# ziqin-h/GIVEPose

Hardware: AMD Instinct MI355X
Metric: images/sec PoseNet fwd, bs=64 256x256 fp16, 1/2/4/8 MI355X; % MFMA roofline (higher is better)
Workload: dtype f16

## Files before the change

### givepose_amd/csrc/gemm.hip

```cpp
#include "common.hpp"

namespace {

struct GemmKP {
    const void* X;
    const void* W;
    const float* bias;
    const float* gamma;
    const void* res;
    void* C;
    float* ws;
    int M, N, K, ldx, ldc, ldres, epi, out_f32;
    int conv, H, Win, Cin, KW, stride, pad, Ho, Wo;
    int tiles_m, tiles_n, nkt, kt_per_split, splitk;
    float* gn_partial;
    int gn_cpg, gn_hw;
    int early;
    const float* ln_stats;
    const float* ln_s;
    int ln_nsl;
    float ln_eps;
    int dbg;
    const char* pf;
    long pf_bytes;
// ... 326 lines not shown
            if (!PRE) {
#pragma unroll
                for (int i = i0; i < i0 + 4; ++i) {
                    const int m = mb + j * 32 + i * 4 + er;
                    for (int e = 0; e < 4; ++e) r4[0][i][e] = 0;
                    if (sres && nok && m < p.M) r4[0][i] = load_res4<RT>(p, m, en);
                }
            }
#pragma unroll
            for (int i = i0; i < i0 + 4; ++i) {
                const int row = i * 4 + er, chunk = lane & 15;
                const f32x4 v = *reinterpret_cast<const f32x4*>(slab + row * 256 + ((chunk ^ (row & 7)) << 4));
                const int m = mb + j * 32 + row;
                if (m < p.M && nok) {
                    const f32x4 o = epi_apply<RT>(epi_code, v, b4, g4, r4[PRE ? j : 0][i]);
                    if (SPL && p.out_planes) {
                        half4 hv, lv;
#pragma unroll
                        for (int e = 0; e < 4; ++e) {
                            hv[e] = (half_t)o[e];
                            lv[e] = (half_t)((o[e] - (float)hv[e]) * p.split_up);
                        }
                        half_t* ch = reinterpret_cast<half_t*>(p.C) + (long)m * p.ldc + en;
                        *reinterpret_cast<half4*>(ch) = hv;
                        *reinterpret_cast<half4*>(ch + p.cplane) = lv;
                    } else
                    if (p.dbg != 4 || o[0] == 12345.678f) store4<RT>(p, m, en, o);
                    if (p.c16) {
                        half4 hv;
#pragma unroll
                        for (int e = 0; e < 4; ++e) hv[e] = (half_t)o[e];
                        *reinterpret_cast<half4*>(reinterpret_cast<half_t*>(p.c16) + (long)m * p.ldc16 + en) = hv;
                    }
                    gsum += (o[0] + o[1]) + (o[2] + o[3]);
                    gsq += (o[0] * o[0] + o[1] * o[1]) + (o[2] * o[2] + o[3] * o[3]);
                }
            }
        }
        if (p.gn_partial && (j & 1)) {
            float a = gsum, q = gsq;
            a += __shfl_xor(a, 16, 64); q += __shfl_xor(q, 16, 64);
            a += __shfl_xor(a, 32, 64); q += __shfl_xor(q, 32, 64);
            if (p.gn_cpg == 8) { a += __shfl_xor(a, 1, 64); q += __shfl_xor(q, 1, 64); }
            const int mrow = mb + (j - 1) * 32;
            if (er == 0 && nok && mrow < p.M && (p.gn_cpg == 4 || (lane & 1) == 0)) {
                const int G = p.N / p.gn_cpg, cpi = p.gn_hw >> 6;
                const int b = mrow / p.gn_hw, ch = (mrow - b * p.gn_hw) >> 6;
                float* o = p.gn_partial + (((long)b * cpi + ch) * G + en / p.gn_cpg) * 2;
                o[0] = a;
                o[1] = q;
            }
            gsum = gsq = 0.f;
        }
    }
}

template <int MT, int NT>
__device__ __forceinline__ void epilogue_split(const GemmKP& p, f32x4 (&acc)[NT][MT], char* slab, int mb, int nb, int lane) {
    switch (p.epi) {
        case GP_EPI_GELU: epilogue_generic<float, MT, NT, true, GP_EPI_GELU>(p, acc, slab, mb, nb, lane); break;
        case GP_EPI_RELU: epilogue_generic<float, MT, NT, true, GP_EPI_RELU>(p, acc, slab, mb, nb, lane); break;
        case GP_EPI_LRELU: epilogue_generic<float, MT, NT, true, GP_EPI_LRELU>(p, acc, slab, mb, nb, lane); break;
        case GP_EPI_SCALE_RES: epilogue_generic<float, MT, NT, true, GP_EPI_SCALE_RES>(p, acc, slab, mb, nb, lane); break;
        case GP_EPI_RES_RELU: epilogue_generic<float, MT, NT, true, GP_EPI_RES_RELU>(p, acc, slab, mb, nb, lane); break;
        default: epilogue_generic<float, MT, NT, true, GP_EPI_NONE>(p, acc, slab, mb, nb, lane); break;
    }
}

template <typename T, int WM, int WN, int MT, int NT, int NS, bool DB = false, int RB = 128, bool PP = false, bool SPL = false, bool R32 = false>
__global__ __launch_bounds__(WM * WN * 64, WM * WN == 4 ? 2 : 1) void gemm_big_kernel(const GemmKP pin) {
    static_assert(NT == 4, "epilogue slab assumes a 64-wide wave tile");
    static_assert(!SPL || sizeof(T) == 2, "split-operand mode: fp16 planes");
    static_assert(!R32 || (sizeof(T) == 2 && !SPL), "R32: fp16 operands with an fp32 residual / output");
    typedef typename std::conditional<SPL || R32, float, T>::type RT;
    GemmKP p = pin;
    int kt0 = 0;
    if constexpr (!PP && !(DB && NS == 2)) {
        if (pin.splitk > 1) {
            kt0 = blockIdx.y * pin.kt_per_split;
            p.nkt = min(pin.nkt - kt0, pin.kt_per_split);
            p.C = reinterpret_cast<float*>(pin.C) + (long)blockIdx.y * pin.M * pin.N;
        }
    }
    static_assert(!PP || (WM * WN == 8 && (NS == 4 || NS == 5) && RB == 64 && !DB), "ping-pong schedule: 8 waves, 4/5-stage ring of 64-byte K steps");
    constexpr int NW = WM * WN;
    constexpr int BM = WM * MT * 16, BN = WN * NT * 16;
    static_assert(RB == 128 || (RB == 64 && !DB), "RB");
    constexpr int EPT = 16 / sizeof(T), KPT = RB / sizeof(T), CPR = RB / 16, RPI = 1024 / RB;
    constexpr int XI = BM / RPI / NW, WI = BN / RPI / NW;
    constexpr int STAGE = (BM + BN) * RB;
    static_assert(NS * STAGE >= NW * 8192, "epilogue slabs must fit");
    __shared__ __attribute__((aligned(1024))) char smem[NS * STAGE];

    const int tid = threadIdx.x, lane = tid & 63;
    const int wave = __builtin_amdgcn_readfirstlane(tid >> 6);
    const int wm = wave % WM, wn = wave / WM;

    const int nblk = p.tiles_m * p.tiles_n;
    const int bid = blockIdx.x;
    const int q = nblk >> 3, r8 = nblk & 7, xcd = bid & 7, idx = bid >> 3;
    const int tile = (xcd < r8 ? xcd * (q + 1) : r8 * (q + 1) + (xcd - r8) * q) + idx;
    const int tm = tile / p.tiles_n, tn = tile - tm * p.tiles_n;
    const int m0 = tm * BM, n0 = tn * BN;
    const PfSink pfs = prefetch_issue(p, bid + blockIdx.y * gridDim.x, gridDim.x * gridDim.y, wave, WM * WN, lane);

    const T* __restrict__ X = reinterpret_cast<const T*>(p.X);
    const T* __restrict__ W = reinterpret_cast<const T*>(p.W);
    const T* zero = reinterpret_cast<const T*>(gp_zero_page_tu);

    const int lrow = lane / CPR;
    const int lchunk = RB == 128 ? ((lane & 7) ^ (lrow & 7)) : ((lane & 3) ^ ((-(lrow >> 2)) & 3));
    const char* xptr[XI];
    unsigned xmask[XI];
    const char* wptr[WI];
#pragma unroll
    for (int i = 0; i < XI; ++i) {
        const int m = m0 + (i * NW + wave) * RPI + lrow;
        const bool ok = m < p.M;
        if (p.conv) {
            const int hw = p.Ho * p.Wo;
            const int b = m / hw, r = m - b * hw;
            const int ho = r / p.Wo, wo = r - ho * p.Wo;
            const int hi0 = ho * p.stride - p.pad, wi0 = wo * p.stride - p.pad;
            xptr[i] = reinterpret_cast<const char*>(X + (((long)b * p.H + hi0) * p.Win + wi0) * p.Cin + lchunk * EPT);
            unsigned mk = 0;
            const int KH = p.K / (p.KW * p.Cin);
            for (int kh = 0; kh < KH; ++kh)
                for (int kw = 0; kw < p.KW; ++kw)
                    if (ok && (unsigned)(hi0 + kh) < (unsigned)p.H && (unsigned)(wi0 + kw) < (unsigned)p.Win)
                        mk |= 1u << (kh * p.KW + kw);
            xmask[i] = mk;
        } else {
            xptr[i] = reinterpret_cast<const char*>(X + (long)m * p.ldx + lchunk * EPT);
            xmask[i] = ok ? 1u : 0u;
        }
    }
#pragma unroll
    for (int i = 0; i < WI; ++i) {
        const int n = n0 + (i * NW + wave) * RPI + lrow;
        wptr[i] = n < p.N ? reinterpret_cast<const char*>(W + (long)n * p.K + lchunk * EPT) : nullptr;
    }
    const int cpt = p.conv ? p.Cin / KPT : 1;

    const unsigned lds0 = (unsigned)(size_t)(lds_char_t*)smem;
    auto stage = [&](int buf, int kt) {
        const unsigned xs = lds0 + buf * STAGE + wave * 1024;
        const unsigned ws = xs + BM * RB;
        long xoff;
        unsigned bit = 1u;
        kt += kt0;
        long xadd = 0, wadd = 0;
        if constexpr (SPL) {
            const int seg = (kt >= p.split_n1 ? 1 : 0) + (kt >= 2 * p.split_n1 ? 1 : 0);
            kt -= seg * p.split_n1;
            xadd = seg == 1 ? p.xplane_b : 0;
            wadd = seg == 0 ? p.wplane_b : 0;
        }
        if (p.conv) {
            const int tap = kt / cpt;
            const int kh = tap / p.KW, kw = tap - kh * p.KW;
            xoff = (((long)kh * p.Win + kw) * p.Cin + (kt - tap * cpt) * KPT) * (long)sizeof(T);
            bit = 1u << tap;
        } else {
            xoff = (long)kt * RB;
        }
        const char* zp = reinterpret_cast<const char*>(zero);
#pragma unroll
// ... 2 lines not shown
        for (int i = 0; i < WI; ++i) glds16(wptr[i] ? wptr[i] + (long)kt * RB + wadd : zp, ws + i * NW * 1024);
    };

    bool lean = false;
    if constexpr (sizeof(T) == 2 && !SPL) {
        const bool res_epi = p.epi == GP_EPI_SCALE_RES || p.epi == GP_EPI_RES_RELU;
        lean = !p.out_f32 && p.dbg != 5 && m0 + BM <= p.M && n0 + BN <= p.N && p.ldc % 8 == 0 &&
               ((size_t)p.C & 15) == 0 && !(res_epi && (p.gn_partial || p.ldres % 8 || ((size_t)p.res & 15)));
    }
    f32x4 acc[NT][MT];
#pragma unroll
    for (int a = 0; a < NT; ++a) {
        f32x4 init = f32x4{0.f, 0.f, 0.f, 0.f};
        if (lean && p.bias && p.epi != GP_EPI_LNFOLD_GELU) init = *reinterpret_cast<const f32x4*>(p.bias + n0 + wn * NT * 16 + a * 16 + (lane >> 4) * 4);
#pragma unroll
        for (int b = 0; b < MT; ++b) acc[a][b] = init;
    }
    auto split_rescale = [&](int kt) {
        if constexpr (SPL) {
            if (kt + kt0 == 2 * p.split_n1) {
#pragma unroll
                for (int a = 0; a < NT; ++a)
#pragma unroll
                    for (int b = 0; b < MT; ++b) acc[a][b] *= p.split_scale;
            }
        }
    };

    const int fr = lane & 15, fq = lane >> 4, sw = fr & 7;
    const int xfo = (wm * MT * 16 + fr) * RB, wfo = (wn * NT * 16 + fr) * RB;
    auto compute = [&](int buf) {
        const char* xs = smem + buf * STAGE + xfo;
        const char* ws = smem + buf * STAGE + BM * RB + wfo;
        if constexpr (RB == 64) {
            const int co = (fq ^ ((-(fr >> 2)) & 3)) << 4;
            uint4 xf[MT], wf[NT];
#pragma unroll
            for (int t = 0; t < NT; ++t) wf[t] = *reinterpret_cast<const uint4*>(ws + t * 1024 + co);
#pragma unroll
            for (int t = 0; t < MT; ++t) xf[t] = *reinterpret_cast<const uint4*>(xs + t * 1024 + co);
#pragma unroll
            for (int mt = 0; mt < MT; ++mt)
#pragma unroll
                for (int nt = 0; nt < NT; ++nt) mma<T>(acc[nt][mt], wf[nt], xf[mt]);
        } else if constexpr (DB) {
            const int co0 = ((0 * 4 + fq) ^ sw) << 4, co1 = ((1 * 4 + fq) ^ sw) << 4;
            uint4 xf0[MT], wf0[NT], xf1[MT], wf1[NT];
#pragma unroll
            for (int t = 0; t < NT; ++t) wf0[t] = *reinterpret_cast<const uint4*>(ws + t * 2048 + co0);
#pragma unroll
            for (int t = 0; t < MT; ++t) xf0[t] = *reinterpret_cast<const uint4*>(xs + t * 2048 + co0);
#pragma unroll
            for (int t = 0; t < NT; ++t) wf1[t] = *reinterpret_cast<const uint4*>(ws + t * 2048 + co1);
#pragma unroll
            for (int t = 0; t < MT; ++t) xf1[t] = *reinterpret_cast<const uint4*>(xs + t * 2048 + co1);
            __builtin_amdgcn_s_setprio(1);
#pragma unroll
            for (int mt = 0; mt < MT; ++mt)
#pragma unroll
                for (int nt = 0; nt < NT; ++nt) mma<T>(acc[nt][mt], wf0[nt], xf0[mt]);
#pragma unroll
            for (int mt = 0; mt < MT; ++mt)
#pragma unroll
                for (int nt = 0; nt < NT; ++nt) mma<T>(acc[nt][mt], wf1[nt], xf1[mt]);
            __builtin_amdgcn_s_setprio(0);
        } else {
#pragma unroll
            for (int ks = 0; ks < 2; ++ks) {
                const int co = ((ks * 4 + fq) ^ sw) << 4;
                uint4 xf[MT], wf[NT];
#pragma unroll
                for (int t = 0; t < NT; ++t) wf[t] = *reinterpret_cast<const uint4*>(ws + t * 2048 + co);
#pragma unroll
                for (int t = 0; t < MT; ++t) xf[t] = *reinterpret_cast<const uint4*>(xs + t * 2048 + co);
#pragma unroll
                for (int mt = 0; mt < MT; ++mt)
#pragma unroll
                    for (int nt = 0; nt < NT; ++nt) mma<T>(acc[nt][mt], wf[nt], xf[mt]);
            }
        }
    };

    constexpr int G = XI + WI;
    if constexpr (PP) {
        constexpr int LEAD = NS - 2;
        const int grp = wave >> 2;
        const int co = (fq ^ ((-(fr >> 2)) & 3)) << 4;
        uint4 xf[MT], wf[NT];
        const bool sdma = !p.conv && (long)BM * p.ldx * sizeof(T) < (1l << 31) && (long)BN * p.K * sizeof(T) < (1l << 31);
        unsigned xo[XI], wo[WI];
#pragma unroll
        for (int i = 0; i < XI; ++i) {
            const int r = min((i * NW + wave) * RPI + lrow, p.M - 1 - m0);
            xo[i] = (unsigned)(((long)r * p.ldx + lchunk * EPT) * sizeof(T));
        }
#pragma unroll
        for (int i = 0; i < WI; ++i) {
            const int r = min((i * NW + wave) * RPI + lrow, p.N - 1 - n0);
            wo[i] = (unsigned)(((long)r * p.K + lchunk * EPT) * sizeof(T));
        }
        const char* xtile = reinterpret_cast<const char*>(X + (long)m0 * p.ldx);
        const char* wtile = reinterpret_cast<const char*>(W + (long)n0 * p.K);
        auto stage_s = [&](int buf, int kt) {
            const unsigned xs = lds0 + buf * STAGE + wave * 1024;
            const unsigned ws = xs + BM * RB;
            long xadd = 0, wadd = 0;
            if constexpr (SPL) {
                const int seg = (kt >= p.split_n1 ? 1 : 0) + (kt >= 2 * p.split_n1 ? 1 : 0);
                kt -= seg * p.split_n1;
                xadd = seg == 1 ? p.xplane_b : 0;
                wadd = seg == 0 ? p.wplane_b : 0;
            }
            const char* bx = xtile + (long)kt * RB + xadd;
            const char* bw = wtile + (long)kt * RB + wadd;
#pragma unroll
            for (int i = 0; i < XI; ++i) glds16_s(bx, xo[i], xs + i * NW * 1024);
#pragma unroll
            for (int i = 0; i < WI; ++i) glds16_s(bw, wo[i], ws + i * NW * 1024);
        };
#pragma unroll
        for (int i = 0; i < LEAD; ++i)
            if (i < p.nkt) { if (sdma) stage_s(i, i); else stage(i, i); }
        if constexpr (LEAD == 3) {
            if (p.nkt >= 3) asm volatile("s_waitcnt vmcnt(%0)" ::"n"(2 * G) : "memory");
            else if (p.nkt == 2) asm volatile("s_waitcnt vmcnt(%0)" ::"n"(G) : "memory");
            else asm volatile("s_waitcnt vmcnt(0)" ::: "memory");
        } else {
            if (p.nkt >= 2) asm volatile("s_waitcnt vmcnt(%0)" ::"n"(G) : "memory");
            else asm volatile("s_waitcnt vmcnt(0)" ::: "memory");
        }
        prefetch_retire(pfs);
        __builtin_amdgcn_s_barrier();
        if (grp) __builtin_amdgcn_s_barrier();
        int buf = 0, nbuf = LEAD;
        clk_stamp(p, 0);
#ifdef GP_PP_STAMPS
#define GP_PPS(k)                                                                                                              \
        do {                                                                                                                     \
            if (p.ws && p.splitk <= 1 && blockIdx.x == 0 && (wave & 3) == 0 && lane == 0 && kt >= 8 && kt < 24) {                  \
                __builtin_amdgcn_sched_barrier(0);                                                                               \
                unsigned long long t_;                                                                                           \
                asm volatile("s_memtime %0\n\ts_waitcnt lgkmcnt(0)" : "=s"(t_) :: "memory");                                    \
                reinterpret_cast<unsigned long long*>(p.ws)[4096 + ((wave >> 2) * 16 + (kt - 8)) * 8 + (k)] = t_;                 \
                __builtin_amdgcn_sched_barrier(0);                                                                               \
            }                                                                                                                    \
        } while (0)
#else
#define GP_PPS(k) do {} while (0)
#endif
        for (int kt = 0; kt < p.nkt; ++kt) {
            GP_PPS(0);
            if (p.dbg != 2) {
                const char* xs = smem + buf * STAGE + xfo;
                const char* ws = smem + buf * STAGE + BM * RB + wfo;
#pragma unroll
                for (int t = 0; t < NT; ++t) wf[t] = *reinterpret_cast<const uint4*>(ws + t * 1024 + co);
#pragma unroll
                for (int t = 0; t < MT; ++t) xf[t] = *reinterpret_cast<const uint4*>(xs + t * 1024 + co);
            }
            __builtin_amdgcn_sched_barrier(0);
            GP_PPS(1);
            if (kt + LEAD < p.nkt && (p.dbg != 1 || kt + LEAD < NS)) { if (sdma) stage_s(nbuf, kt + LEAD); else stage(nbuf, kt + LEAD); }
            GP_PPS(2);
            if (LEAD == 3 && kt + 3 < p.nkt) asm volatile("s_waitcnt vmcnt(%0)" ::"n"(2 * G) : "memory");
            else if (kt + 2 < p.nkt) asm volatile("s_waitcnt vmcnt(%0)" ::"n"(G) : "memory");
            else asm volatile("s_waitcnt vmcnt(0)" ::: "memory");
// ... 1098 lines not shown
    }
    GP_SM(KMAX);
#undef GP_SM
}


template <int MR>
__global__ __launch_bounds__(256) void gemv_kernel(const GemmKP p) {
    constexpr int KC = 4096, NCH = KC / 512;
    __shared__ __attribute__((aligned(16))) half_t xs[MR][KC];
    const int tid = threadIdx.x, lane = tid & 63, wave = tid >> 6;
    const int n0 = blockIdx.x * 8 + wave * 2;
    const half_t* X = reinterpret_cast<const half_t*>(p.X);
    const half_t* W0 = reinterpret_cast<const half_t*>(p.W) + (long)n0 * p.K + lane * 8;
    float acc[MR][2];
#pragma unroll
    for (int m = 0; m < MR; ++m) acc[m][0] = acc[m][1] = 0.f;
    for (int k0 = 0; k0 < p.K; k0 += KC) {
        const int kc = min(KC, p.K - k0), nch = kc >> 9;
        uint4 w[2][NCH];
#pragma unroll
        for (int j = 0; j < NCH; ++j)
            if (j < nch) {
                w[0][j] = *reinterpret_cast<const uint4*>(W0 + k0 + j * 512);
                w[1][j] = *reinterpret_cast<const uint4*>(W0 + p.K + k0 + j * 512);
            }
        if (k0) __syncthreads();
        for (int i = tid; i < MR * (kc >> 3); i += 256) {
            const int m = i / (kc >> 3), c = i - m * (kc >> 3);
            uint4 v = uint4{0u, 0u, 0u, 0u};
            if (m < p.M) v = *reinterpret_cast<const uint4*>(X + (long)m * p.ldx + k0 + c * 8);
            *reinterpret_cast<uint4*>(&xs[m][c * 8]) = v;
        }
        __syncthreads();
#pragma unroll
        for (int j = 0; j < NCH; ++j)
            if (j < nch) {
#pragma unroll
                for (int m = 0; m < MR; ++m) {
                    const uint4 xv = *reinterpret_cast<const uint4*>(&xs[m][j * 512 + lane * 8]);
                    const unsigned xw[4] = {xv.x, xv.y, xv.z, xv.w};
#pragma unroll
                    for (int c = 0; c < 2; ++c) {
                        const unsigned ww[4] = {w[c][j].x, w[c][j].y, w[c][j].z, w[c][j].w};
#pragma unroll
                        for (int e = 0; e < 4; ++e)
                            acc[m][c] = __builtin_amdgcn_fdot2(__builtin_bit_cast(half2v, xw[e]), __builtin_bit_cast(half2v, ww[e]), acc[m][c], false);
                    }
                }
            }
    }
#pragma unroll
    for (int m = 0; m < MR; ++m)
#pragma unroll
        for (int c = 0; c < 2; ++c)
#pragma unroll
            for (int o = 32; o >= 1; o >>= 1) acc[m][c] += __shfl_xor(acc[m][c], o, 64);
    if (lane == 0) {
        const f32x4 z = f32x4{0.f, 0.f, 0.f, 0.f};
#pragma unroll
        for (int m = 0; m < MR; ++m)
            if (m < p.M) {
                const f32x4 b = p.bias ? f32x4{p.bias[n0], p.bias[n0 + 1], 0.f, 0.f} : z;
                const f32x4 v = epi_apply<half_t>(p.epi, f32x4{acc[m][0], acc[m][1], 0.f, 0.f}, b, z, half4{0, 0, 0, 0});
                if (p.out_f32) {
                    float* o = reinterpret_cast<float*>(p.C) + (long)m * p.ldc + n0;
                    o[0] = v[0];
                    o[1] = v[1];
                } else {
                    half_t* o = reinterpret_cast<half_t*>(p.C) + (long)m * p.ldc + n0;
                    o[0] = (half_t)v[0];
                    o[1] = (half_t)v[1];
                }
            }
    }
}

}

static bool pp_enabled() {
    static const bool on = [] { const char* e = getenv("GP_GEMM_PP"); return !(e && e[0] == '0'); }();
    return on;
}

static bool conv_wide_enabled() {
    static const bool on = [] { const char* e = getenv("GP_CONV_WIDE"); return !(e && e[0] == '0'); }();
    return on;
}

static bool conv_window_enabled() {
    static const bool on = [] { const char* e = getenv("GP_CONV_WINDOW"); return !(e && e[0] == '0'); }();
    return on;
}

static long pp_min_k() {
    static const long k = [] { const char* e = getenv("GP_PP_MIN_K"); return e ? atol(e) : 512l; }();
    return k;
}

static int gp_num_cus() {
    static const int n = [] {
        int dev = 0, cu = 0;
        if (hipGetDevice(&dev) != hipSuccess || hipDeviceGetAttribute(&cu, hipDeviceAttributeMultiprocessorCount, dev) != hipSuccess || cu <= 0) cu = 256;
        return cu;
    }();
    return n;
}

static bool prefetch_enabled() {
    static const bool on = [] { const char* e = getenv("GP_GEMM_PREFETCH"); return !(e && e[0] == '0'); }();
    return on;
}

static bool wreg_enabled() {
    static const bool on = [] { const char* e = getenv("GP_GEMM_WREG"); return !(e && e[0] == '0'); }();
    return on;
}
static bool wreg_early() {
    static const bool on = [] { const char* e = getenv("GP_GEMM_WREG_EARLY"); return !(e && e[0] == '0'); }();
    return on;
}
static long wreg_min_rows() {
    static const long k = [] { const char* e = getenv("GP_GEMM_WREG_MIN_ROWS"); return e ? atol(e) : 6144l; }();
    return k;
}

static int wreg_variant() {
    static const int v = [] { const char* e = getenv("GP_GEMM_WREG_VARIANT"); const int x = e ? atoi(e) : (gp_gelu16_enabled() ? 21 : 22); return (x >= 19 && x <= 22) ? x : 17; }();
    return v;
}

static long co_min_tiles() {
    static const long k = [] { const char* e = getenv("GP_GEMM_CO_MIN_TILES"); return e ? atol(e) : 32l; }();
    return k;
}

static double smallm_tile_bias() {
    static const double b = [] { const char* e = getenv("GP_GEMM_SMALLM_BIAS"); return e ? atof(e) : 0.0; }();
    return b;
}
static double smallm_estimate(int M, int N, int K, int mt) {
    const double wgs = (double)(M / (16 * mt)) * (N / 32), kb_per_wg = (16.0 * mt + 32.0) * K * 2.0 / 1024.0;
    const double one = 1.0 + kb_per_wg / 60.0, many = wgs / 256.0 * kb_per_wg / 45.0;
    return 2.6 + (one > many ? one : many) + (mt == 4 ? 1.5 : 0.0);
}

static bool gemv_enabled() {
    static const bool on = [] { const char* e = getenv("GP_GEMM_GEMV"); return !(e && e[0] == '0'); }();
    return on;
}

static int smallm_max_rows() {
    static const int n = [] { const char* e = getenv("GP_GEMM_SMALLM_MAXROWS"); return e && atoi(e) > 0 ? atoi(e) : 16384; }();
    return n;
}

static bool smallm_enabled() {
    static const bool on = [] { const char* e = getenv("GP_GEMM_SMALLM"); return !(e && e[0] == '0'); }();
    return on;
}

static long pp_min_tiles() {
    const char* e = getenv("GP_GEMM_PP_MIN_TILES");
    return e ? atol(e) : 192;
}

// ... 188 lines not shown
        switch (d->epilogue) {
            case GP_EPI_GELU:
#ifdef GP_WREG_STAMPS
                if (p.dbg == 16 && p.ws) { hipLaunchKernelGGL((gemm_wreg_kernel<GP_EPI_GELU, 16>), dim3(grid), dim3(512), 0, s, p); break; }
                if (p.dbg == 1) { hipLaunchKernelGGL((gemm_wreg_kernel<GP_EPI_GELU, 1>), dim3(grid), dim3(512), 0, s, p); break; }
                if (p.dbg == 2) { hipLaunchKernelGGL((gemm_wreg_kernel<GP_EPI_GELU, 2>), dim3(grid), dim3(512), 0, s, p); break; }
                if (p.dbg == 4) { hipLaunchKernelGGL((gemm_wreg_kernel<GP_EPI_GELU, 4>), dim3(grid), dim3(512), 0, s, p); break; }
                if (p.dbg == 8) { hipLaunchKernelGGL((gemm_wreg_kernel<GP_EPI_NONE, 8>), dim3(grid), dim3(512), 0, s, p); break; }
                if (p.dbg == 10) { hipLaunchKernelGGL((gemm_wreg_kernel<GP_EPI_NONE, 10>), dim3(grid), dim3(512), 0, s, p); break; }
                if (p.dbg == 14) { hipLaunchKernelGGL((gemm_wreg_kernel<GP_EPI_NONE, 14>), dim3(grid), dim3(512), 0, s, p); break; }
#endif
                hipLaunchKernelGGL(gemm_wreg_kernel<GP_EPI_GELU>, dim3(grid), dim3(512), 0, s, p);
                break;
            case GP_EPI_RELU: hipLaunchKernelGGL(gemm_wreg_kernel<GP_EPI_RELU>, dim3(grid), dim3(512), 0, s, p); break;
            case GP_EPI_LRELU: hipLaunchKernelGGL(gemm_wreg_kernel<GP_EPI_LRELU>, dim3(grid), dim3(512), 0, s, p); break;
            default: hipLaunchKernelGGL(gemm_wreg_kernel<GP_EPI_NONE>, dim3(grid), dim3(512), 0, s, p); break;
        }
        GP_LAUNCH_CHECK("gp_gemm");
    }
    if (variant == 17) {
        GP_REQUIRE(wreg_ok && d->ldc % 8 == 0 && ((size_t)d->C & 15) == 0, "gp_gemm: variant 17 needs a plain fp16 GEMM with K = 512, N %% 256 == 0, M %% 32 == 0, ldc %% 8 == 0, "
                   "16-byte aligned C, epilogue none/gelu/relu/lrelu");
        const int nsl = d->N / 256, tiles = d->M / 32;
        const int want = gp_num_cus() / nsl > 0 ? gp_num_cus() / nsl : 1;
        p.tiles_m = cdiv(tiles, want);
        const int groups = cdiv(tiles, p.tiles_m);
        const int grid = cdiv(groups * nsl, 8) * 8;
        switch (d->epilogue) {
            case GP_EPI_GELU: hipLaunchKernelGGL(gemm_wreg2_kernel<GP_EPI_GELU>, dim3(grid), dim3(512), 0, s, p); break;
            case GP_EPI_RELU: hipLaunchKernelGGL(gemm_wreg2_kernel<GP_EPI_RELU>, dim3(grid), dim3(512), 0, s, p); break;
            case GP_EPI_LRELU: hipLaunchKernelGGL(gemm_wreg2_kernel<GP_EPI_LRELU>, dim3(grid), dim3(512), 0, s, p); break;
            default: hipLaunchKernelGGL(gemm_wreg2_kernel<GP_EPI_NONE>, dim3(grid), dim3(512), 0, s, p); break;
        }
        GP_LAUNCH_CHECK("gp_gemm");
    }
    if (variant >= 19 && variant <= 22) {
        GP_REQUIRE(wreg_ok && d->ldc % 8 == 0 && ((size_t)d->C & 15) == 0, "gp_gemm: variant 19-22 needs a plain fp16 GEMM with K = 512, N %% 256 == 0, M %% 32 == 0, ldc %% 8 == 0, "
                   "16-byte aligned C, epilogue none/gelu/relu/lrelu");
        const int nsl = d->N / 256, tiles = d->M / 32;
        const int want = gp_num_cus() / nsl > 0 ? gp_num_cus() / nsl : 1;
        p.tiles_m = cdiv(tiles, want);
        const int groups = cdiv(tiles, p.tiles_m);
        const int grid = cdiv(groups * nsl, 8) * 8;
        const bool s32 = variant <= 20, g16 = variant == 20 || variant == 21;
#define GP_W3(E, S, G) hipLaunchKernelGGL((gemm_wreg3_kernel<E, S, G>), dim3(grid), dim3(512), 0, s, p)
        switch (d->epilogue) {
            case GP_EPI_GELU:
                if (s32) { if (g16) GP_W3(GP_EPI_GELU, 1, 1); else GP_W3(GP_EPI_GELU, 1, 0); }
                else { if (g16) GP_W3(GP_EPI_GELU, 0, 1); else GP_W3(GP_EPI_GELU, 0, 0); }
                break;
            case GP_EPI_RELU: if (s32) GP_W3(GP_EPI_RELU, 1, 0); else GP_W3(GP_EPI_RELU, 0, 0); break;
            case GP_EPI_LRELU: if (s32) GP_W3(GP_EPI_LRELU, 1, 0); else GP_W3(GP_EPI_LRELU, 0, 0); break;
            default: if (s32) GP_W3(GP_EPI_NONE, 1, 0); else GP_W3(GP_EPI_NONE, 0, 0); break;
        }
#undef GP_W3
        GP_LAUNCH_CHECK("gp_gemm");
    }
    if (variant == 13) {
        GP_REQUIRE(win_ok, "gp_gemm: variant 13 needs a 3x3 s1 p1 fp16 conv with Cout 256, W in {64, 32, 16}");
        p.tiles_m = d->M / 256;
        p.tiles_n = 1;
        const bool wide = !split && d->Win >= 32 && d->M % 512 == 0 && d->H % (512 / d->Win) == 0 && p.dbg != 9 && (p.dbg == 8 || conv_wide_enabled());
        if (split) {
            if (d->Win == 64) hipLaunchKernelGGL((conv3_pp_kernel<64, 4, true>), dim3(p.tiles_m), dim3(512), 0, s, p);
            else if (d->Win == 32) hipLaunchKernelGGL((conv3_pp_kernel<32, 4, true>), dim3(p.tiles_m), dim3(512), 0, s, p);
            else hipLaunchKernelGGL((conv3_pp_kernel<16, 4, true>), dim3(p.tiles_m), dim3(512), 0, s, p);
        }
#ifdef GP_CONV_GNL
        else if (d->Win == 64 && p.dbg == 7) hipLaunchKernelGGL((conv3_pp_kernel<64, 4, false, true>), dim3(p.tiles_m), dim3(512), 0, s, p);
        else if (d->Win == 32 && p.dbg == 7) hipLaunchKernelGGL((conv3_pp_kernel<32, 4, false, true>), dim3(p.tiles_m), dim3(512), 0, s, p);
#endif
        else if (wide && d->Win == 64) { p.tiles_m = d->M / 512; hipLaunchKernelGGL((conv3_pp_kernel<64, 4, false, false, true>), dim3(p.tiles_m * 2), dim3(512), 0, s, p); }
        else if (wide && d->Win == 32) { p.tiles_m = d->M / 512; hipLaunchKernelGGL((conv3_pp_kernel<32, 4, false, false, true>), dim3(p.tiles_m * 2), dim3(512), 0, s, p); }
        else if (d->Win == 64) hipLaunchKernelGGL((conv3_pp_kernel<64, 4>), dim3(p.tiles_m), dim3(512), 0, s, p);
        else if (d->Win == 32) hipLaunchKernelGGL((conv3_pp_kernel<32, 4>), dim3(p.tiles_m), dim3(512), 0, s, p);
        else hipLaunchKernelGGL((conv3_pp_kernel<16, 4>), dim3(p.tiles_m), dim3(512), 0, s, p);
        GP_LAUNCH_CHECK("gp_gemm");
    }
    if (variant == 12) {
        if (d->dtype == GP_F16) launch_big<half_t, 2, 4, 8, 4, 5, false, 64, true>(p, s); else launch_big<float, 2, 2, 4, 4, 2>(p, s);
        GP_LAUNCH_CHECK("gp_gemm");
    }
    if (variant == 10) {
        if (split) launch_big<half_t, 2, 4, 8, 4, 4, false, 64, true, true>(p, s);
        else if (r32) launch_big<half_t, 2, 4, 8, 4, 4, false, 64, true, false, true>(p, s);
        else if (d->dtype == GP_F16) launch_big<half_t, 2, 4, 8, 4, 4, false, 64, true>(p, s); else launch_big<float, 2, 2, 4, 4, 2>(p, s);
        GP_LAUNCH_CHECK("gp_gemm");
    }
    if (variant == 11) {
        if (d->dtype == GP_F16) launch_big<half_t, 2, 4, 4, 4, 4, false, 64, true>(p, s); else launch_big<float, 2, 2, 4, 4, 2>(p, s);
        GP_LAUNCH_CHECK("gp_gemm");
    }
    if (variant == 8) {
        if (split) launch_big<half_t, 2, 2, 8, 4, 3, false, 64, false, true>(p, s);
        else if (d->dtype == GP_F16) launch_big<half_t, 2, 2, 8, 4, 3, false, 64>(p, s); else launch_big<float, 2, 2, 4, 4, 2>(p, s);
        GP_LAUNCH_CHECK("gp_gemm");
    }
    if (variant == 9) {
        if (d->dtype == GP_F16) launch_big<half_t, 2, 2, 8, 4, 4, false, 64>(p, s); else launch_big<float, 2, 2, 4, 4, 2>(p, s);
        GP_LAUNCH_CHECK("gp_gemm");
    }
    if (variant == 7) {
        if (split) launch_big<half_t, 2, 2, 4, 4, 2, true, 128, false, true>(p, s);
        else if (r32) launch_big<half_t, 2, 2, 4, 4, 2, true, 128, false, false, true>(p, s);
        else if (d->dtype == GP_F16) launch_big<half_t, 2, 2, 4, 4, 2, true>(p, s); else launch_big<float, 2, 2, 4, 4, 2>(p, s);
        GP_LAUNCH_CHECK("gp_gemm");
    }
    if (variant == 5) {
        if (d->dtype == GP_F16) launch_big<half_t, 2, 2, 4, 4, 4>(p, s); else launch_big<float, 2, 2, 4, 4, 4>(p, s);
        GP_LAUNCH_CHECK("gp_gemm");
    }
    if (variant == 4) {
        if (p.splitk > 1) {
            GemmKP q = p;
            q.C = d->workspace; q.out_f32 = 1; q.ldc = d->N; q.epi = GP_EPI_NONE; q.bias = nullptr; q.gamma = nullptr; q.res = nullptr;
            if (split) launch_big<half_t, 2, 2, 4, 4, 2, false, 128, false, true>(q, s);
            else if (d->dtype == GP_F16) launch_big<half_t, 2, 2, 4, 4, 2>(q, s); else launch_big<float, 2, 2, 4, 4, 2>(q, s);
            p.splitk = q.splitk;
            const long work = (long)d->M * (d->N / 4);
            if (d->dtype == GP_F16 && !split) hipLaunchKernelGGL(splitk_reduce_kernel<half_t>, dim3(cdiv(work, 256)), dim3(256), 0, s, p);
            else hipLaunchKernelGGL(splitk_reduce_kernel<float>, dim3(cdiv(work, 256)), dim3(256), 0, s, p);
            GP_LAUNCH_CHECK("gp_gemm");
        }
        if (split) launch_big<half_t, 2, 2, 4, 4, 2, false, 128, false, true>(p, s);
        else if (d->dtype == GP_F16) launch_big<half_t, 2, 2, 4, 4, 2>(p, s); else launch_big<float, 2, 2, 4, 4, 2>(p, s);
        GP_LAUNCH_CHECK("gp_gemm");
    }
    if (variant == 3) {
        if (d->dtype == GP_F16) launch_big<half_t, 2, 4, 8, 4, 2>(p, s); else launch_big<float, 2, 2, 4, 4, 2>(p, s);
        GP_LAUNCH_CHECK("gp_gemm");
    }
    if (variant == 2) {
        if (d->dtype == GP_F16) launch_big<half_t, 4, 2, 4, 4, 3>(p, s); else launch_big<float, 4, 2, 4, 4, 3>(p, s);
        GP_LAUNCH_CHECK("gp_gemm");
    }
    return gp_fail(GP_ERR_INVALID, "gp_gemm: variant %d not handled", variant);
}
```

Measured before the change: 12800.

## Add eight-phase ping-pong GEMM schedule with double-buffered 128-byte K steps

Adds a new ping-pong path to the big fp16 GEMM kernel. It runs on two LDS buffers of 128-byte K steps, split into half-tiles, and works through four compute quadrants per K tile. Fragment reads, global-to-LDS staging and MFMA bursts are interleaved under barriers and priority hints. Plain fp16 GEMMs with K >= 1024 use it by default, with an environment switch and debug overrides. The goal is to hide more load latency and cut barrier overhead per K step, at the cost of more registers, a tighter schedule and more code paths.

```diff
diff --git a/givepose_amd/csrc/gemm.hip b/givepose_amd/csrc/gemm.hip
--- a/givepose_amd/csrc/gemm.hip
+++ b/givepose_amd/csrc/gemm.hip
@@ -432,7 +432,8 @@
             p.C = reinterpret_cast<float*>(pin.C) + (long)blockIdx.y * pin.M * pin.N;
         }
     }
-    static_assert(!PP || (WM * WN == 8 && (NS == 4 || NS == 5) && RB == 64 && !DB), "ping-pong schedule: 8 waves, 4/5-stage ring of 64-byte K steps");
+    static_assert(!PP || (WM * WN == 8 && (NS == 4 || NS == 5) && RB == 64 && !DB) || (WM == 2 && WN == 4 && MT == 8 && NS == 2 && RB == 128 && !DB && !SPL && !R32 && sizeof(T) == 2),
+                  "ping-pong schedule: 8 waves, 4/5-stage ring of 64-byte K steps, or the eight-phase schedule on two buffers of 128-byte K steps");
     constexpr int NW = WM * WN;
     constexpr int BM = WM * MT * 16, BN = WN * NT * 16;
     static_assert(RB == 128 || (RB == 64 && !DB), "RB");
@@ -601,6 +602,110 @@
     };
 
     constexpr int G = XI + WI;
+    if constexpr (PP && RB == 128) {
+        constexpr int HT = 128 * RB;
+        static_assert(STAGE == 4 * HT, "two buffers of four half-tiles");
+        const int grp = wave >> 2;
+        unsigned xo[2][2], wo[2][2];
+#pragma unroll
+        for (int h = 0; h < 2; ++h)
+#pragma unroll
+            for (int j = 0; j < 2; ++j) {
+                const int r = (j * NW + wave) * RPI + lrow;
+                const int xr = min((r >> 6) * 128 + h * 64 + (r & 63), p.M - 1 - m0);
+                const int wr = min((r >> 5) * 64 + h * 32 + (r & 31), p.N - 1 - n0);
+                xo[h][j] = (unsigned)(((long)xr * p.ldx + lchunk * EPT) * sizeof(T));
+                wo[h][j] = (unsigned)(((long)wr * p.K + lchunk * EPT) * sizeof(T));
+            }
+        const char* xtile = reinterpret_cast<const char*>(X + (long)m0 * p.ldx);
+        const char* wtile = reinterpret_cast<const char*>(W + (long)n0 * p.K);
+        auto stage_x = [&](int b, int h, int kt) __attribute__((always_inline)) {
+            const char* bx = xtile + (long)kt * RB;
+            const unsigned ls = lds0 + b * STAGE + h * HT + wave * 1024;
+            glds16_s(bx, xo[h][0], ls);
+            glds16_s(bx, xo[h][1], ls + NW * 1024);
+        };
+        auto stage_w = [&](int b, int h, int kt) __attribute__((always_inline)) {
+            const char* bw = wtile + (long)kt * RB;
+            const unsigned ls = lds0 + b * STAGE + (2 + h) * HT + wave * 1024;
+            glds16_s(bw, wo[h][0], ls);
+            glds16_s(bw, wo[h][1], ls + NW * 1024);
+        };
+        const int co0 = (fq ^ sw) << 4, co1 = ((4 + fq) ^ sw) << 4;
+        const char* xfb = smem + (wm * 64 + fr) * RB;
+        const char* wfb = smem + 2 * HT + (wn * 32 + fr) * RB;
+        uint4 xf[2][4][2], wf[2][2][2];
+        auto read_x = [&](int b, int h) __attribute__((always_inline)) {
+#pragma unroll
+            for (int t = 0; t < 4; ++t) {
+                xf[h][t][0] = *reinterpret_cast<const uint4*>(xfb + b * STAGE + h * HT + t * 16 * RB + co0);
+                xf[h][t][1] = *reinterpret_cast<const uint4*>(xfb + b * STAGE + h * HT + t * 16 * RB + co1);
+            }
+        };
+        auto read_w = [&](int b, int h) __attribute__((always_inline)) {
+#pragma unroll
+            for (int t = 0; t < 2; ++t) {
+                wf[h][t][0] = *reinterpret_cast<const uint4*>(wfb + b * STAGE + h * HT + t * 16 * RB + co0);
+                wf[h][t][1] = *reinterpret_cast<const uint4*>(wfb + b * STAGE + h * HT + t * 16 * RB + co1);
+            }
+        };
+        auto quadrant = [&](int xh, int wh) __attribute__((always_inline)) {
+            __builtin_amdgcn_sched_barrier(0);
+            __builtin_amdgcn_s_barrier();
+            asm volatile("s_waitcnt lgkmcnt(0)" ::: "memory");
+            __builtin_amdgcn_sched_barrier(0);
+            __builtin_amdgcn_s_setprio(1);
+#pragma unroll
+            for (int ks = 0; ks < 2; ++ks)
+#pragma unroll
+                for (int mt = 0; mt < 4; ++mt)
+#pragma unroll
+                    for (int nt = 0; nt < 2; ++nt) mma<T>(acc[wh * 2 + nt][xh * 4 + mt], wf[wh][nt][ks], xf[xh][mt][ks]);
+            __builtin_amdgcn_s_setprio(0);
+            __builtin_amdgcn_sched_barrier(0);
+            __builtin_amdgcn_s_barrier();
+            __builtin_amdgcn_sched_barrier(0);
+        };
+        auto ktile = [&](int b, int kt, bool s1, bool s2) __attribute__((always_inline)) {
+            read_w(b, 0);
+            __builtin_amdgcn_sched_barrier(0);
+            read_x(b, 0);
+            __builtin_amdgcn_sched_barrier(0);
+            if (s1) stage_x(b ^ 1, 1, kt + 1);
+            asm volatile("s_waitcnt lgkmcnt(8)" ::: "memory");
+            quadrant(0, 0);
+            read_w(b, 1);
+            __builtin_amdgcn_sched_barrier(0);
+            if (s2) stage_w(b, 0, kt + 2);
+            quadrant(0, 1);
+            read_x(b, 1);
+            __builtin_amdgcn_sched_barrier(0);
+            if (s2) stage_x(b, 0, kt + 2);
+            quadrant(1, 0);
+            if (s2) {
+                stage_w(b, 1, kt + 2);
+                asm volatile("s_waitcnt vmcnt(6)" ::: "memory");
+            } else {
+                asm volatile("s_waitcnt vmcnt(0)" ::: "memory");
+            }
+            quadrant(1, 1);
+        };
+        stage_x(0, 0, 0); stage_w(0, 0, 0); stage_w(0, 1, 0); stage_x(0, 1, 0);
+        stage_w(1, 0, 1); stage_x(1, 0, 1); stage_w(1, 1, 1);
+        asm volatile("s_waitcnt vmcnt(6)" ::: "memory");
+        prefetch_retire(pfs);
+        __builtin_amdgcn_s_barrier();
+        if (grp) __builtin_amdgcn_s_barrier();
+        clk_stamp(p, 0);
+        for (int kt = 0; kt + 2 < p.nkt; kt += 2) {
+            ktile(0, kt, true, true);
+            ktile(1, kt + 1, true, true);
+        }
+        ktile(0, p.nkt - 2, true, false);
+        ktile(1, p.nkt - 1, false, false);
+        clk_stamp(p, 1);
+        if (!grp) __builtin_amdgcn_s_barrier();
+    } else
     if constexpr (PP) {
         constexpr int LEAD = NS - 2;
         const int grp = wave >> 2;
@@ -1865,6 +1970,13 @@
     static const bool on = [] { const char* e = getenv("GP_GEMM_PP"); return !(e && e[0] == '0'); }();
     return on;
 }
+
+static bool pp128_enabled() {
+    static const bool on = [] { const char* e = getenv("GP_GEMM_PP128"); return !(e && e[0] == '0'); }();
+    return on;
+}
+
+static bool pp128_wins(int K) { return K >= 1024; }
 
 static bool conv_wide_enabled() {
     static const bool on = [] { const char* e = getenv("GP_CONV_WIDE"); return !(e && e[0] == '0'); }();
@@ -2219,6 +2331,21 @@
         GP_LAUNCH_CHECK("gp_gemm");
     }
     if (variant == 10) {
+        const int force = p.dbg == 11 ? 1 : p.dbg == 12 ? -1 : 0;
+        if (force) p.dbg = 0;
+        const bool pp128_ok = d->dtype == GP_F16 && !split && !r32 && d->KH == 0 && d->K % 128 == 0 && d->K >= 256 &&
+                              256l * d->ldx * 2 < (1l << 31) && 256l * d->K * 2 < (1l << 31);
+        GP_REQUIRE(force != 1 || pp128_ok, "gp_gemm: variant 1110 (eight-phase schedule) needs a plain fp16 GEMM (no conv, split-operand mode or fp32 residual), "
+                   "K %% 128 == 0, K >= 256 (got K=%d)", d->K);
+#ifdef GP_PP_STAMPS
+        const bool dbg_ok = false;
+#else
+        const bool dbg_ok = p.dbg == 0 || (p.dbg >= 3 && p.dbg <= 5);
+#endif
+        if (force == 1 || (force == 0 && dbg_ok && pp128_ok && pp128_enabled() && pp128_wins(d->K))) {
+            launch_big<half_t, 2, 4, 8, 4, 2, false, 128, true>(p, s);
+            GP_LAUNCH_CHECK("gp_gemm/pp128");
+        }
         if (split) launch_big<half_t, 2, 4, 8, 4, 4, false, 64, true, true>(p, s);
         else if (r32) launch_big<half_t, 2, 4, 8, 4, 4, false, 64, true, false, true>(p, s);
         else if (d->dtype == GP_F16) launch_big<half_t, 2, 4, 8, 4, 4, false, 64, true>(p, s); else launch_big<float, 2, 2, 4, 4, 2>(p, s);
```

New measurement: 13150 (median of 6 runs). 1.03x the previous value.
